# csxmli2016/MARCONet

Measured on AMD Instinct MI355X. Metric: SR images/sec (32x512 LR -> 128x2048 SR), higher is better.
Workload: dtype f16x2; 1 GPU; metric config: batch 256 x 32x512 LR, 16 glyphs/img, enc+TSPGAN+TSPSRNet, fp16x2; per_gpu_batch=256, global_batch=256, glyphs_per_image=16, parallelism=dp1, precision_mode=fp16x2, need_prior_image=True, prior_image_precision=fp16, weights=synthetic:tame, collective=none

## Files before the change

### marconet_amd/_lib.py

```python
import ctypes
import os

_HERE = os.path.dirname(os.path.abspath(__file__))
LIB_PATH = os.environ.get("MARCONET_HIP_LIB", os.path.join(_HERE, "lib", "libmarconet_hip.so"))

ABI_VERSION = 4
MNET_F32, MNET_F16, MNET_F16X2, MNET_F16M = 0, 1, 2, 3
ACT_NONE, ACT_RELU, ACT_LRELU, ACT_LRELU_SQRT2, ACT_TANH, ACT_GELU, ACT_SIGMOID = range(7)
ALGO_AUTO, ALGO_REG_STAGED, ALGO_LDS_DMA, ALGO_SKINNY, ALGO_DMA_CFG0, ALGO_STRIP_CFG0, ALGO_DMA_CFG16, ALGO_FLAG_ONE_TILE = 0, 1, 2, 3, 16, 32, 64, 256
ALGO_FLAG_X1_CENTER = 512
ALGO_FLAG_SHUFFLE2 = 1024

c_int, c_void_p, c_float, c_double, c_i64 = ctypes.c_int32, ctypes.c_void_p, ctypes.c_float, ctypes.c_double, ctypes.c_int64


class ConvDesc(ctypes.Structure):
    _fields_ = [
        ("dtype", c_int),
        ("x0", c_void_p), ("c0", c_int),
        ("x1", c_void_p), ("c1", c_int),
        ("n", c_int), ("h", c_int), ("w", c_int),
        ("wgt", c_void_p),
        ("cout", c_int), ("kh", c_int), ("kw", c_int), ("stride_h", c_int), ("stride_w", c_int),
        ("pad_h", c_int), ("pad_w", c_int),
# ... 34 lines not shown


class CmpStats(ctypes.Structure):
    _fields_ = [("max_abs_diff", c_float), ("max_abs_ref", c_float), ("max_abs_mode", c_float), ("reserved", c_int),
                ("argmax_index", c_i64), ("sum_sq_diff", c_double), ("sum_sq_ref", c_double),
                ("nonfinite_mode", c_i64), ("nonfinite_ref", c_i64)]


CMP_WG_ELEMS, CMP_MAX_SLICES = 2048, 32


def cmp_slices(elems_per_group):
    return max(1, min(CMP_MAX_SLICES, -(-int(elems_per_group) // CMP_WG_ELEMS)))


def cmp_workspace_bytes(n_groups, elems_per_group):
    return int(n_groups) * cmp_slices(elems_per_group) * ctypes.sizeof(CmpStats)


def cmp_records(raw):
    raw = bytes(memoryview(raw).cast("B")) if not isinstance(raw, (bytes, bytearray)) else bytes(raw)
    n = ctypes.sizeof(CmpStats)
    if len(raw) % n:
        raise ValueError("cmp_records: %d bytes are no whole number of %d-byte records" % (len(raw), n))
    return [CmpStats.from_buffer_copy(raw, k) for k in range(0, len(raw), n)]


SYMBOLS = {
    "mnet_last_error": (ctypes.c_char_p, []),
    "mnet_abi_version": (c_int, []),
    "mnet_conv2d_nhwc": (c_int, [ctypes.POINTER(ConvDesc), c_void_p]),
    "mnet_conv2d_nhwc_ex": (c_int, [ctypes.POINTER(ConvDesc), c_int, c_void_p]),
    "mnet_conv2d_splitk": (c_int, [ctypes.POINTER(ConvDesc), c_int, c_void_p, c_void_p]),
    "mnet_conv2d_plan": (c_int, [ctypes.POINTER(ConvDesc), c_int]),
    "mnet_conv2d_flops": (c_double, [ctypes.POINTER(ConvDesc)]),
    "mnet_nchw_to_nhwc": (c_int, [c_void_p, c_void_p, c_int, c_int, c_int, c_int, c_int, c_int, c_void_p]),
    "mnet_nhwc_to_nchw": (c_int, [c_void_p, c_int, c_void_p, c_int, c_int, c_int, c_int, c_int, c_void_p]),
    "mnet_upsample2x_nhwc": (c_int, [c_void_p, c_void_p, c_int, c_int, c_int, c_int, c_int, c_void_p]),
    "mnet_upsample2x_scale_nhwc": (c_int, [c_void_p, c_void_p, c_int, c_int, c_int, c_int, c_int, c_void_p, c_void_p]),
    "mnet_upsample2x_convert_nhwc": (c_int, [c_void_p, c_int, c_void_p, c_int, c_int, c_int, c_int, c_int, c_void_p, c_void_p]),
    "mnet_affine_act_nhwc": (c_int, [c_void_p, c_void_p, c_int, c_int, c_int, c_int, c_void_p, c_void_p, c_int, c_void_p]),
    "mnet_groupnorm_affine": (c_int, [c_void_p, c_int, c_int, c_int, c_int, c_int, c_void_p, c_void_p, c_void_p,
                                      c_float, c_void_p, c_int, c_void_p, c_void_p, c_void_p]),
    "mnet_groupnorm_affine_from_partial": (c_int, [c_void_p, c_int, c_int, c_int, c_int, c_void_p, c_void_p, c_void_p, c_float, c_void_p, c_void_p, c_void_p]),
    "mnet_polyphase_ring_fix": (c_int, [c_void_p, c_void_p, c_void_p, c_void_p, c_void_p, c_int, c_int, c_int, c_int, c_int, c_void_p, c_void_p]),
    "mnet_groupnorm_affine_from_partial_ring": (c_int, [c_void_p, c_void_p, c_int, c_int, c_int, c_int, c_void_p, c_void_p, c_float, c_void_p, c_void_p, c_void_p]),
    "mnet_adain_crop_concat": (c_int, [c_void_p, c_void_p, c_void_p, c_int, c_int, c_int, c_int, c_int,
                                       c_void_p, c_void_p, c_void_p, c_void_p, c_void_p]),
    "mnet_adain_crop_concat_gn": (c_int, [c_void_p, c_void_p, c_void_p, c_int, c_int, c_int, c_int, c_int,
                                          c_void_p, c_void_p, c_void_p, c_void_p, c_void_p, c_void_p, c_float, c_void_p, c_void_p, c_void_p]),
    "mnet_adain_crop_concat_split": (c_int, [c_void_p, c_void_p, c_void_p, c_int, c_int, c_int, c_int, c_int,
                                             c_void_p, c_void_p, c_void_p, c_void_p, c_void_p, c_void_p, c_float, c_void_p, c_void_p,
                                             c_void_p, c_void_p, c_int, c_void_p]),
    "mnet_glyph_scatter_affine": (c_int, [c_void_p, c_void_p, c_void_p, c_void_p, c_int, c_int, c_int, c_int, c_int,
                                          c_void_p, c_void_p, c_void_p, c_void_p]),
    "mnet_layernorm": (c_int, [c_void_p, c_void_p, c_void_p, c_void_p, c_int, c_int, c_float, c_void_p]),
    "mnet_token_mix": (c_int, [c_void_p, c_void_p, c_void_p, c_void_p, c_void_p, c_void_p, c_int, c_int, c_int,
                               c_int, c_float, c_void_p]),
    "mnet_attention": (c_int, [c_void_p, c_void_p, c_int, c_int, c_int, c_float, c_void_p]),
    "mnet_pixelnorm": (c_int, [c_void_p, c_void_p, c_int, c_int, c_void_p]),
    "mnet_embed_gather": (c_int, [c_void_p, c_void_p, c_void_p, c_int, c_int, c_int, c_int, c_int, c_void_p]),
    "mnet_embed_gather_scaled": (c_int, [c_void_p, c_void_p, c_void_p, c_void_p, c_int, c_int, c_int, c_int, c_int, c_void_p]),
    "mnet_demod": (c_int, [c_void_p, c_void_p, c_void_p, c_int, c_int, c_int, c_void_p]),
    "mnet_argmax_rows": (c_int, [c_void_p, c_void_p, c_int, c_int, c_void_p]),
    "mnet_convert": (c_int, [c_void_p, c_int, c_void_p, c_int, c_i64, c_void_p]),
    "mnet_fused_bias_act": (c_int, [c_void_p, c_void_p, c_void_p, c_i64, c_int, c_int, c_float, c_float, c_void_p]),
    "mnet_torgb": (c_int, [c_void_p, c_int, c_int, c_int, c_int, c_int, c_void_p, c_void_p, c_void_p, c_void_p, c_void_p, c_void_p, c_void_p]),
    "mnet_conv3x3_rgb": (c_int, [c_void_p, c_int, c_int, c_int, c_int, c_int, c_void_p, c_void_p, c_int, c_void_p, c_void_p, c_void_p]),
    "mnet_sr_postprocess": (c_int, [c_void_p, c_int, c_void_p, c_int, c_i64, c_int, c_void_p]),
    "mnet_nonfinite_flag": (c_int, [c_void_p, c_int, c_i64, c_void_p, c_void_p]),
    "mnet_compare_stats": (c_int, [c_void_p, c_int, c_void_p, c_int, c_int, c_i64, c_void_p, c_void_p, c_void_p]),
    "mnet_lq_from_u8": (c_int, [c_void_p, c_void_p, c_int, c_int, c_int, c_void_p, c_int, c_void_p]),
    "mnet_panel_u8": (c_int, [c_void_p, c_int, c_void_p, c_int, c_void_p, c_void_p, c_void_p, c_int, c_int, c_void_p, c_void_p]),
    "mnet_stitch_u8": (c_int, [c_void_p, c_int, c_int, c_int, c_void_p, c_void_p, c_int, c_int, c_void_p, c_void_p]),
    "mnet_paste_u8": (c_int, [c_void_p, c_int, c_int, c_int, c_void_p, c_int, c_void_p, c_int, c_int, c_void_p]),
    "mnet_pack_weights": (c_int, [c_void_p, c_int, c_int, c_int, c_int, c_void_p, c_void_p, c_float, c_int, c_int, c_int, c_void_p,
                                  c_void_p, c_void_p]),
    "mnet_pack_wsq": (c_int, [c_void_p, c_int, c_int, c_int, c_float, c_void_p, c_void_p]),
    "mnet_demod_scaled": (c_int, [c_void_p, c_void_p, c_void_p, c_int, c_int, c_int, c_void_p, c_void_p]),
    "mnet_style_rows": (c_int, [c_void_p, c_int, c_int, c_int, c_int, c_void_p, c_int, c_void_p, c_void_p, c_void_p, c_int, c_void_p]),
    "mnet_gather_rows": (c_int, [c_void_p, c_int, c_int, c_int, c_int, c_void_p, c_int, c_void_p, c_void_p]),
}

_lib = None


class MarconetHipError(RuntimeError):
    """Raised for a non-zero C-ABI status; test_sr.py's ``try/except ... continue`` (:181-190) still works."""


def load():
    global _lib
    if _lib is not None:
        return _lib
    if not os.path.isfile(LIB_PATH):
        raise ImportError(
            "marconet_amd: %s not found — build it with `python -c 'import __graft_entry__ as g; g.build()'` "
            "or marconet_amd/csrc/build.sh (there is no CPU/eager fallback)" % LIB_PATH)
    lib = ctypes.CDLL(LIB_PATH)
    for name, (res, args) in SYMBOLS.items():
        fn = getattr(lib, name)
        fn.restype = res
        fn.argtypes = args
    if lib.mnet_abi_version() != ABI_VERSION:
        raise ImportError("marconet_amd: ABI version mismatch in %s" % LIB_PATH)
    _lib = lib
    return lib


def check(status, what):
    if status != 0:
        msg = load().mnet_last_error()
        raise MarconetHipError("%s failed (status %d): %s" % (what, status, msg.decode() if msg else "?"))
```

### marconet_amd/networks.py

```python
import math
import os

import torch
import torch.nn as nn

from . import _lib, ops
from .glyphs import GlyphTables
from .packing import (MX_DTYPE, PRECISIONS, SPLIT_DTYPE, PackCache, is_split, default_precision, equal_linear_scale, pack_conv_weight,
                      pack_linear_weight, pack_polyphase_conv_weight, pack_vec, pack_wsq, padded_cout, rgb_pad, torch_dtype)
from .resnet import resnet45stride as resnet45
from .textvit_arch import TextViT as TextEncoder

_STYLE_NORM = not bool(int(os.environ.get("MNET_NO_STYLE_NORM", "0")))
_FOLD_SKIP = not bool(int(os.environ.get("MNET_NO_FOLD_SKIP", "0")))
_NO_POLYPHASE = os.environ.get("MNET_NO_POLYPHASE", "0") == "1"
_POLYPHASE_CONV_UP = os.environ.get("MNET_POLYPHASE_CONV_UP", "0") == "1"
_FUSE_IMG_CONVERT = os.environ.get("MNET_NO_FUSE_IMG_CONVERT", "0") != "1"
_FUSE_CONV1_MOD = os.environ.get("MNET_NO_FUSE_CONV1_MOD", "0") != "1"
RGB_PAD = 8


class _Precision:
    def set_precision(self, precision):
        if precision not in PRECISIONS:
            raise ValueError("precision must be one of %s" % ", ".join(PRECISIONS))
        self.precision = precision
        for m in self.children():
            if hasattr(m, "precision"):
                m.precision = precision
        return self


class TextContextEncoderV2(nn.Module, _Precision):

    def __init__(self, dim=512, num_classes=6736):
        super().__init__()
        self.resnet = resnet45()
        self.transformer = TextEncoder(num_classes=num_classes, dim=512, max_length=16)
        self.set_precision(default_precision())

    @staticmethod
    def resnet_precision(precision):
        return "fp16x3" if precision == "fp16x2" else precision

    def set_precision(self, precision):
        _Precision.set_precision(self, precision)
        self.resnet.precision = self.resnet_precision(precision)
        return self

    def forward(self, lq, *, precision=None):
        with torch.no_grad(), ops.on_device(lq):
            rp = self.resnet_precision(self.precision if precision is None else precision)
            dtype = torch_dtype(rp)
            x = ops.nchw_to_nhwc(lq.contiguous().float(), dtype, c_ld=rgb_pad(dtype))
            feat = self.resnet.forward_nhwc(x, rp)
            feat = ops.convert(feat, torch.float32)
            return self.transformer.forward_nhwc(feat)


class PixelNorm(nn.Module):
    pass


class EqualLinear(nn.Module):
    def __init__(self, in_channels, out_channels, bias=True, bias_init_val=0, lr_mul=1, activation=None):
        super().__init__()
        self.in_channels, self.out_channels, self.lr_mul, self.activation = in_channels, out_channels, lr_mul, activation
        self.scale = equal_linear_scale(in_channels, lr_mul)
        self.weight = nn.Parameter(torch.randn(out_channels, in_channels).div_(lr_mul))
        if bias:
            self.bias = nn.Parameter(torch.zeros(out_channels).fill_(bias_init_val))
        else:
            self.register_parameter("bias", None)


class SelectText(nn.Module):
    def __init__(self, class_num, channel, size=4):
        super().__init__()
        self.size = size
        self.TextEmbeddings = nn.Parameter(torch.randn(class_num, channel, 1, 1))


class ModulatedConv2d(nn.Module):
    def __init__(self, in_channel, out_channel, kernel_size, style_dim, demodulate=True, upsample=False,
                 downsample=False, blur_kernel=(1, 3, 3, 1)):
        super().__init__()
        self.eps = 1e-8
        self.kernel_size, self.in_channel, self.out_channel = kernel_size, in_channel, out_channel
        self.upsample, self.downsample, self.demodulate = upsample, downsample, demodulate
        self.scale = 1 / math.sqrt(in_channel * kernel_size ** 2)
        self.padding = kernel_size // 2
        self.weight = nn.Parameter(torch.randn(1, out_channel, in_channel, kernel_size, kernel_size))
        self.modulation = EqualLinear(style_dim, in_channel, bias=True, bias_init_val=1, lr_mul=1, activation=None)


class FusedLeakyReLU(nn.Module):

    def __init__(self, channel, negative_slope=0.2, scale=2 ** 0.5):
        super().__init__()
        self.bias = nn.Parameter(torch.zeros(channel))
        self.negative_slope, self.scale = negative_slope, scale


class StyledConv(nn.Module):
    def __init__(self, in_channel, out_channel, kernel_size, style_dim, upsample=False, blur_kernel=(1, 3, 3, 1),
                 demodulate=True):
        super().__init__()
        self.conv = ModulatedConv2d(in_channel, out_channel, kernel_size, style_dim, upsample=upsample,
                                    blur_kernel=blur_kernel, demodulate=demodulate)
        self.bias = nn.Parameter(torch.zeros(1, out_channel, 1, 1))
        self.activate = FusedLeakyReLU(out_channel)


class ToRGB(nn.Module):
    def __init__(self, in_channel, style_dim, upsample=True, blur_kernel=(1, 3, 3, 1)):
        super().__init__()
        self.upsample = upsample
        self.conv = ModulatedConv2d(in_channel, 3, 1, style_dim, demodulate=False)
        self.bias = nn.Parameter(torch.zeros(1, 3, 1, 1))


def returned_image_precision(mode):
    return "fp16x3" if mode == "fp16x2" else None


class TextGenerator(nn.Module):

    def __init__(self, size, style_dim, n_mlp, class_num, channel_multiplier=1, blur_kernel=(1, 3, 3, 1), lr_mlp=0.01):
        super().__init__()
        self.size, self.n_mlp, self.style_dim, self.class_num = size, n_mlp, style_dim, class_num
        self.style_mlp = nn.Sequential(PixelNorm(), *[
            EqualLinear(style_dim, style_dim, bias=True, bias_init_val=0, lr_mul=lr_mlp, activation="fused_lrelu")
            for _ in range(n_mlp)])
        cm = channel_multiplier
        self.channels = {4: 512, 8: 512, 16: 512, 32: 512, 64: 256 * cm, 128: 128 * cm, 256: 64 * cm, 512: 32 * cm,
                         1024: 16 * cm}
        self.input_text = SelectText(class_num, self.channels[4])
        self.conv1 = StyledConv(self.channels[4], self.channels[4], 3, style_dim, blur_kernel=blur_kernel)
        self.to_rgb1 = ToRGB(self.channels[4], style_dim, upsample=False)
        self.log_size = int(math.log(size, 2))
        self.convs, self.upsamples, self.to_rgbs = nn.ModuleList(), nn.ModuleList(), nn.ModuleList()
        cin = self.channels[4]
        for i in range(3, self.log_size + 1):
            cout = self.channels[2 ** i]
            self.convs.append(StyledConv(cin, cout, 3, style_dim, upsample=True, blur_kernel=blur_kernel))
            self.convs.append(StyledConv(cout, cout, 3, style_dim, blur_kernel=blur_kernel))
            self.to_rgbs.append(ToRGB(cout, style_dim))
            cin = cout
        self.n_latent = self.log_size * 2 - 2
        self.precision = default_precision()
        self.module_call_fp16x3 = True
        self._cache = PackCache()

    def _build(self, dtype):
        pk = {}
        f = lambda t: t.detach().float().contiguous()
        pk["mlp"] = []
        for i in range(1, self.n_mlp + 1):
            el = self.style_mlp[i]
            pk["mlp"].append((pack_linear_weight(el.weight, el.scale), f(el.bias.detach() * el.lr_mul)))
        pk["emb"] = f(self.input_text.TextEmbeddings.detach().reshape(self.class_num, -1))

        def styled(sc):
            mc = sc.conv
            w0 = mc.weight.detach()[0]
            return dict(cin=mc.in_channel, cout=mc.out_channel, up=mc.upsample,
                        w=pack_conv_weight(w0, dtype, scale=mc.scale),
                        wsq_t=pack_wsq(w0, mc.scale),
                        mod_w=pack_linear_weight(mc.modulation.weight, mc.modulation.scale), mod_b=f(mc.modulation.bias),
                        bias=f(sc.bias.detach().reshape(-1) + sc.activate.bias.detach()))

        def torgb(tr):
            mc = tr.conv
            return dict(cin=mc.in_channel, w=pack_conv_weight(mc.weight.detach()[0], torch.float32, cin_mult=1, cout_mult=1, scale=mc.scale).reshape(3, -1).contiguous(),
                        mod_w=pack_linear_weight(mc.modulation.weight, mc.modulation.scale), mod_b=f(mc.modulation.bias),
                        bias=pack_vec(tr.bias, 4))

        pk["conv1"] = styled(self.conv1)
        pk["rgb1"] = torgb(self.to_rgb1)
        pk["convs"] = [styled(c) for c in self.convs]
        pk["rgbs"] = [torgb(t) for t in self.to_rgbs]
        layers = [pk["conv1"], pk["rgb1"]] + pk["convs"] + pk["rgbs"]
        off = 0
        for L in layers:
            L["mod_off"] = off
            off += L["cin"]
        pk["mod_all_w"] = torch.cat([L["mod_w"] for L in layers], dim=0).contiguous()
        pk["mod_all_b"] = torch.cat([L["mod_b"] for L in layers], dim=0).contiguous()
        pk["mod_total"] = off
        return pk

    @staticmethod
    def _mod(mod, L, per_glyph=True, bcast=0):
        S, idx = mod[0], mod[1] if per_glyph else None
        if _STYLE_NORM:
            return ops.style_rows(S, L["mod_off"], L["cin"], idx, bcast)
        return ops.gather_rows(S, L["mod_off"], L["cin"], idx), None, None

    @classmethod
    def _style(cls, mod, L):
        s, eps, _ = cls._mod(mod, L)
        if mod[1] is None:
            return s, ops.demod(s, L["wsq_t"], eps)
        su, eps_u, _ = cls._mod(mod, L, per_glyph=False)
        return s, ops.gather_rows(ops.demod(su, L["wsq_t"], eps_u), idx=mod[1])

    @staticmethod
    def _styled(L, x, s, d, premodulated, post=None, out=None):
        return ops.conv2d(x, L["w"], L["cout"], 3, 3, (1, 1), (1, 1), in_scale=None if premodulated else s,
                          out_scale=d, bias=L["bias"], act=ops.ACT_LRELU_SQRT2, post_scale=post, out=out)

    @classmethod
    def _to_rgb(cls, mod, L, x, skip):
        s, _, sb = cls._mod(mod, L, bcast=1)
        return ops.torgb(x, L["w"], s, sb, L["bias"], skip)

    def forward_nhwc(self, styles, labels, need_image=True, style_index=None, p64_out=None, p32_out=None, image_precision=None,
                     precision=None):
        precision = self.precision if precision is None else precision
        pk = self._cache.get(self, precision, self._build)
        dtype = torch_dtype(precision)
        pk_img = pk if image_precision in (None, precision) else self._cache.get(self, image_precision, self._build)
        lat = ops.pixelnorm(styles)
        for w, b in pk["mlp"]:
            lat = ops.linear(lat, w, self.style_dim, bias=b, act=ops.ACT_LRELU_SQRT2)
        mod = (ops.linear(lat, pk["mod_all_w"], pk["mod_total"], bias=pk["mod_all_b"]), style_index)
        s, d = self._style(mod, pk["conv1"])
        x = ops.embed_gather(pk["emb"], labels, dtype, self.class_num, scale=s if _FUSE_CONV1_MOD else None)
        x = self._styled(pk["conv1"], x, s, d, premodulated=_FUSE_CONV1_MOD)
        skip = self._to_rgb(mod, pk["rgb1"], x, None) if need_image else None
        p64 = p32 = None
        for lvl in range(len(pk["rgbs"])):
            if not need_image and p64 is not None and p32 is not None:
                return None, p64, p32
            pkl, up_dtype = pk, None
            if pk_img is not pk and p64 is not None and p32 is not None:
                pkl = pk_img
                up_dtype = torch_dtype(image_precision)
                if not (_FUSE_IMG_CONVERT and up_dtype == torch.float16 and is_split(x.dtype)):
                    x = ops.convert(x, up_dtype)
            La, Lb = pkl["convs"][2 * lvl], pkl["convs"][2 * lvl + 1]
            sa, da = self._style(mod, La)
            sb, db = self._style(mod, Lb)
            xu = ops.upsample2x(x, scale=sa, out_dtype=up_dtype if up_dtype != x.dtype else None)
            xa = self._styled(La, xu, sa, da, premodulated=True, post=sb)
            del xu
            wx = xa.shape[2]
            x = self._styled(Lb, xa, sb, db, premodulated=True, out=p64_out if wx == 64 else (p32_out if wx == 32 else None))
            del xa
            if need_image:
                skip = self._to_rgb(mod, pk["rgbs"][lvl], x, skip)
            if x.shape[2] == 64:
                p64 = x
            if x.shape[2] == 32:
                p32 = x
        if p64 is None or p32 is None:
            raise RuntimeError("no generator level is 64 / 32 pixels wide for %d characters per sample "
                               "(models/networks.py:155-160 selects the prior levels by absolute width)" % labels.shape[1])
        return skip, p64, p32

    def forward(self, styles, labels, noise=None, *, precision=None):
        with torch.no_grad(), ops.on_device(styles):
            styles = styles.contiguous().float()
            labels = labels.to(styles.device).contiguous().long()
            if labels.dim() != 2 or labels.shape[0] != styles.shape[0]:
                raise ValueError("labels must be [N,c] with N == styles.size(0)")
            if labels.numel() and (int(labels.min()) < 0 or int(labels.max()) >= self.class_num):
                raise RuntimeError("label index out of range [0,%d)" % self.class_num)
            mode = self.precision if precision is None else precision
            if mode == "fp16x2" and self.module_call_fp16x3:
                mode = "fp16x3"
            img, p64, p32 = self.forward_nhwc(styles, labels, precision=mode)
            out = ops.nhwc_to_nchw(img, c=3), ops.nhwc_to_nchw(p64), ops.nhwc_to_nchw(p32)
            out[1]._mnet_nhwc, out[2]._mnet_nhwc = (p64, out[1]._version, out[1].data_ptr()), (p32, out[2]._version, out[2].data_ptr())
            return out


class TSPGAN(nn.Module, _Precision):
    def __init__(self, out_size=128, num_style_feat=512, class_num=6736, num_mlp=8):
        super().__init__()
        self.TextGenerator = TextGenerator(size=out_size, style_dim=num_style_feat, n_mlp=num_mlp, class_num=class_num)
        self.precision = default_precision()

    def forward(self, styles, labels, noise):
        return self.TextGenerator(styles, labels, noise, precision=self.precision)


class _SNConv(nn.Module):

    def __init__(self, cin, cout, k=3, stride=1):
        super().__init__()
        self.in_channels, self.out_channels, self.kernel_size, self.stride = cin, cout, k, stride
        conv = nn.Conv2d(cin, cout, k, stride, k // 2)
        self.bias = nn.Parameter(conv.bias.detach().clone())
        self.weight_orig = nn.Parameter(conv.weight.detach().clone())
        nrm = lambda t: t / (t.norm() + 1e-12)
        self.register_buffer("weight_u", nrm(torch.randn(cout)))
        self.register_buffer("weight_v", nrm(torch.randn(cin * k * k)))


def GroupNorm(in_channels):
    assert in_channels % 32 == 0
    return nn.GroupNorm(num_groups=in_channels // 32, num_channels=in_channels, eps=1e-6, affine=True)


def _as_rows32(x):
    b, c = x.shape[:2]
    flat = x.contiguous().float().reshape(b * c, -1)
    m = flat.shape[1]
    mp = (m + 31) // 32 * 32
    if mp != m:
        flat = torch.cat([flat, flat.new_zeros((flat.shape[0], mp - m))], dim=1)
    return flat.reshape(b * c, 1, mp // 32, 32), m, mp


def swish(x):
    v = x.contiguous().float().reshape(1, -1)
    m = v.shape[1]
    mp = (m + 31) // 32 * 32
    if mp != m:
        v = torch.cat([v, v.new_zeros((1, mp - m))], dim=1)
    one = torch.ones((1, 32), dtype=torch.float32, device=x.device)
    y = ops.affine_act(v.reshape(1, 1, mp // 32, 32), one, None, swish=True)
    return y.reshape(-1)[:m].reshape(x.shape)


def calc_mean_std_4D(feat, eps=1e-5):
    if feat.dim() != 4:
        raise AssertionError("The input feature should be 4D tensor.")
# ... 268 lines not shown
```

### marconet_amd/ops.py

```python
import ctypes
import functools
import os

import numpy as np
import torch

from . import _lib
from ._lib import (ACT_GELU, ACT_LRELU, ACT_LRELU_SQRT2, ACT_NONE, ACT_RELU, ACT_SIGMOID, ACT_TANH, MNET_F16,
                   MNET_F16M, MNET_F16X2, MNET_F32, ConvDesc)
from .packing import MX_DTYPE, SPLIT_DTYPE, is_split, mx_weight_rows, new_tensor, tag, untag

__all__ = ["conv2d", "linear", "nchw_to_nhwc", "nhwc_to_nchw", "upsample2x", "affine_act", "groupnorm_affine",
           "adain_crop_concat", "adain_crop_concat_gn", "glyph_scatter_affine", "layernorm", "token_mix", "attention", "pixelnorm",
           "embed_gather", "demod", "argmax_rows", "convert", "fused_bias_act", "sr_postprocess", "lq_from_u8", "panel_u8", "paste_u8", "conv3x3_rgb", "torgb", "stats",
           "pack_weights", "pack_wsq", "gather_rows", "style_rows", "nonfinite_flag", "compare_stats", "gn_partial_buffer", "can_emit_gn_partial", "groupnorm_affine_from_partial",
           "polyphase_plan", "upconv3x3_polyphase", "polyphase_ring_fix", "groupnorm_affine_from_partial_ring",
           "ACT_NONE", "ACT_RELU", "ACT_LRELU", "ACT_LRELU_SQRT2", "ACT_TANH", "ACT_GELU", "ACT_SIGMOID"]


def _plumbing(fn):
    @functools.wraps(fn)
    def wrapper(*args, **kwargs):
        with torch._C.DisableTorchFunctionSubclass():
            return fn(*args, **kwargs)
    return wrapper


def _dt(t):
    if t.dtype == torch.float32:
        return MNET_F32
    if t.dtype == torch.float16:
        return MNET_F16
    if t.dtype == SPLIT_DTYPE:
        return MNET_F16X2
    if t.dtype == MX_DTYPE:
        return MNET_F16M
    raise TypeError("marconet_amd: unsupported dtype %s" % t.dtype)


def _p(t):
    return None if t is None else ctypes.c_void_p(t.data_ptr())


def _addr(t):
    return None if t is None else t.data_ptr()


def _stream():
    return ctypes.c_void_p(torch.cuda.current_stream().cuda_stream)


def _need_cuda(*ts):
    cur = None
    for t in ts:
        if t is None:
            continue
        if not t.is_cuda:
            raise RuntimeError("marconet_amd: tensors must live on a HIP device (got %s); there is no CPU path" % t.device)
        if cur is None:
            cur = torch.cuda.current_device()
        if t.device.index != cur:
            raise RuntimeError("marconet_amd: tensor on %s but the current device is cuda:%d — enter torch.cuda.device(...) "
                               "(the nn.Module forwards and MarconetPipeline do)" % (t.device, cur))
        if not t.is_contiguous():
            raise RuntimeError("marconet_amd: non-contiguous tensor passed to a kernel wrapper")


def _raw(t):
    return untag(t).view(torch.float16) if is_split(t.dtype) else t


@_plumbing
def cat_rows(parts):
    if len(parts) == 1:
        return parts[0]
    out = torch.cat([_raw(p) for p in parts], dim=0)
    return tag(out.view(parts[0].dtype)) if is_split(parts[0].dtype) else out


@_plumbing
def take_rows(t, idx):
    out = _raw(t).index_select(0, idx)
    return tag(out.view(t.dtype)) if is_split(t.dtype) else out


def on_device(t):
    if not t.is_cuda:
        raise RuntimeError("marconet_amd: tensors must live on a HIP device (got %s); there is no CPU path" % t.device)
    return torch.cuda.device(t.device)


class _Stats:

    def __init__(self):
        self.enabled = False
        self.timing = False
        self.reset()

    def reset(self):
# ... 174 lines not shown
    scale = torch.empty((n, c), dtype=torch.float32, device=x.device)
    shift = torch.empty((n, c), dtype=torch.float32, device=x.device)
    stats.tail("groupnorm_stats", (x,), lambda: _lib.check(lib.mnet_groupnorm_affine(_p(x), _dt(x), n, h, w, c, _p(valid_w), _p(gamma), _p(beta), eps,
                                                                                  _p(partial), slices, _p(scale), _p(shift), _stream()), "mnet_groupnorm_affine"))
    return scale, shift


def gn_partial_buffer(n, h, w, c, device):
    return torch.empty((n * h * w // 32, c // 32, 2), dtype=torch.float32, device=device)


_PLAN_CACHE = {}
_PLAN_ADDR = 1 << 20


def _align(t):
    return None if t is None else (128 if t.data_ptr() % 128 == 0 else 16 if t.data_ptr() % 16 == 0 else 0)


def conv_plan(x0, cout, kh=1, kw=1, stride=(1, 1), pad=(0, 0), x1=None, act=ACT_NONE, in_scale=False, residual=False, out_scale=False,
              gn_partial=False, x1_center=False, algo=0):
    n, h, w, c0 = x0.shape
    if x1_center:
        algo |= _lib.ALGO_FLAG_X1_CENTER
    key = (_dt(x0), n, h, w, c0, None if x1 is None else x1.shape[3], _align(x0), _align(x1), cout, kh, kw, tuple(stride), tuple(pad), act,
           bool(in_scale), bool(residual), bool(out_scale), bool(gn_partial), algo)
    k = _PLAN_CACHE.get(key)
    if k is None:
        addr = [_PLAN_ADDR if present else None for present in (in_scale, residual, out_scale, gn_partial)]
        d = _conv_desc(x0, x1, cout, kh, kw, stride, pad, wgt=_PLAN_ADDR, y=_PLAN_ADDR, in_scale=addr[0], residual=addr[1], out_scale=addr[2],
                       act=act, gn_partial=addr[3])
        k = int(_lib.load().mnet_conv2d_plan(ctypes.byref(d), algo))
        if k >= 0:
            _PLAN_CACHE[key] = k
    return k


def polyphase_plan(x, c, act=ACT_NONE, gn_partial=True, algo=0):
    if x.dtype != MX_DTYPE:
        return -1
    return conv_plan(x, 4 * c, 3, 3, (1, 1), (1, 1), act=act, gn_partial=gn_partial, algo=algo | _lib.ALGO_FLAG_SHUFFLE2)


@_plumbing
def polyphase_ring_fix(top, bottom, left, right, y):
    lib = _lib.load()
    _need_cuda(top, bottom, left, right, y)
    n, h2, w2, c = y.shape
    if tuple(top.shape) != (n, 4, w2, c) or tuple(bottom.shape) != (n, 4, w2, c) or tuple(left.shape) != (n, h2, 4, c) or tuple(right.shape) != (n, h2, 4, c):
        raise RuntimeError("polyphase_ring_fix: strips %s %s %s %s do not fit y %s" % (tuple(top.shape), tuple(bottom.shape), tuple(left.shape), tuple(right.shape), tuple(y.shape)))
    sums = torch.empty((n, c // 32, 2), dtype=torch.float64, device=y.device)
    stats.tail("polyphase_ring", (top, left, top, left), lambda: _lib.check(lib.mnet_polyphase_ring_fix(_p(top), _p(bottom), _p(left), _p(right), _p(y), _dt(y), n, h2, w2, c,
                                                                                                      _p(sums), _stream()), "mnet_polyphase_ring_fix"))
    return sums


def groupnorm_affine_from_partial_ring(partial, ring_sums, n, h, w, c, gamma, beta, eps=1e-6):
    lib = _lib.load()
    _need_cuda(partial, ring_sums, gamma, beta)
    scale = torch.empty((n, c), dtype=torch.float32, device=partial.device)
    shift = torch.empty((n, c), dtype=torch.float32, device=partial.device)
    _lib.check(lib.mnet_groupnorm_affine_from_partial_ring(_p(partial), _p(ring_sums), n, h, w, c, _p(gamma), _p(beta), eps, _p(scale), _p(shift), _stream()),
               "mnet_groupnorm_affine_from_partial_ring")
    return scale, shift


@_plumbing
def _strip_pair(x, dim):
    r = _raw(x)
    k = r.shape[dim]
    out = torch.cat([r.narrow(dim, 0, 2), r.narrow(dim, k - 2, 2)], dim=0)
    return tag(out.view(x.dtype)) if is_split(x.dtype) else out


def upconv3x3_polyphase(x, wgt_poly, bias_poly, wgt, bias, c, act=ACT_NONE, algo=0, out=None):
    n, h, w, _ = x.shape
    part = gn_partial_buffer(n, h, w, 4 * c, x.device)
    y = conv2d(x, wgt_poly, 4 * c, 3, 3, (1, 1), (1, 1), bias=bias_poly, act=act, gn_partial=part, algo=algo, shuffle2=True, out=out)
    tb = conv2d(upsample2x(_strip_pair(x, 1)), wgt, c, 3, 3, (1, 1), (1, 1), bias=bias, act=act)
    lr = conv2d(upsample2x(_strip_pair(x, 2)), wgt, c, 3, 3, (1, 1), (1, 1), bias=bias, act=act)
    return y, part, polyphase_ring_fix(tb[:n], tb[n:], lr[:n], lr[n:], y)


def plan_is_lds_dma(k):
    return _lib.ALGO_DMA_CFG0 <= k < _lib.ALGO_STRIP_CFG0 or k >= _lib.ALGO_DMA_CFG16


def can_emit_gn_partial(x0, x1, cout, stride, ho, wo, act=ACT_NONE):
    c = x0.shape[3] + (0 if x1 is None else x1.shape[3])
    if not (x0.dtype == MX_DTYPE and tuple(stride) == (1, 1) and cout >= 64 and cout % 32 == 0 and c % 32 == 0 and x0.shape[3] % 32 == 0
            and (ho * wo) % 32 == 0 and not _NO_EPILOGUE_GN):
        return False
    return conv_plan(x0, cout, 3, 3, stride, (1, 1), x1=x1, act=act, gn_partial=True) >= _lib.ALGO_DMA_CFG0


def groupnorm_affine_from_partial(partial, n, h, w, c, gamma, beta, eps=1e-6, valid_w=None):
    lib = _lib.load()
    _need_cuda(partial, gamma, beta, valid_w)
    scale = torch.empty((n, c), dtype=torch.float32, device=partial.device)
    shift = torch.empty((n, c), dtype=torch.float32, device=partial.device)
    _lib.check(lib.mnet_groupnorm_affine_from_partial(_p(partial), n, h, w, c, _p(valid_w), _p(gamma), _p(beta), eps, _p(scale), _p(shift), _stream()),
               "mnet_groupnorm_affine_from_partial")
    return scale, shift


@_plumbing
def adain_crop_concat(prior, feat, g_img, g_x1, g_y1, g_w):
    lib = _lib.load()
    _need_cuda(prior, feat, g_img, g_x1, g_y1, g_w)
    G, S, S2, C = prior.shape
    B, FH, FW, FC = feat.shape
    if S != S2 or FH != S or FC != C or prior.dtype != feat.dtype:
        raise RuntimeError("adain_crop_concat: shape mismatch prior %s feat %s" % (tuple(prior.shape), tuple(feat.shape)))
    out = new_tensor((G, S, S, 2 * C), prior.dtype, prior.device)
    _lib.check(lib.mnet_adain_crop_concat(_p(prior), _p(feat), _p(out), _dt(prior), G, S, C, FW, _p(g_img), _p(g_x1),
                                          _p(g_y1), _p(g_w), _stream()), "mnet_adain_crop_concat")
    return out


_NO_EPILOGUE_GN = os.environ.get("MNET_NO_EPILOGUE_GN", "0") == "1"
ADAIN_SPLIT_BELOW = 256
_ADAIN_SPLIT = {"0": False, "1": True}.get(os.environ.get("MNET_ADAIN_SPLIT", ""))


@_plumbing
def adain_crop_concat_gn(prior, feat, g_img, g_x1, g_y1, g_w, gamma, beta, eps=1e-6, split=None):
    lib = _lib.load()
    _need_cuda(prior, feat, g_img, g_x1, g_y1, g_w, gamma, beta)
    G, S, S2, C = prior.shape
    B, FH, FW, FC = feat.shape
    if S != S2 or FH != S or FC != C or prior.dtype != feat.dtype or gamma.numel() != 2 * C:
        raise RuntimeError("adain_crop_concat_gn: shape mismatch prior %s feat %s" % (tuple(prior.shape), tuple(feat.shape)))
    out = new_tensor((G, S, S, 2 * C), prior.dtype, prior.device)
    scale = torch.empty((G, 2 * C), dtype=torch.float32, device=prior.device)
    shift = torch.empty((G, 2 * C), dtype=torch.float32, device=prior.device)
    if split is None:
        split = _ADAIN_SPLIT if _ADAIN_SPLIT is not None else G < ADAIN_SPLIT_BELOW
    if split:
        slices = 16
        partial = torch.empty((G * slices * C * 4,), dtype=torch.float64, device=prior.device)
        stat = torch.empty((G, 4, C), dtype=torch.float32, device=prior.device)
        stats.tail("adain", (prior, prior, out), lambda: _lib.check(lib.mnet_adain_crop_concat_split(
            _p(prior), _p(feat), _p(out), _dt(prior), G, S, C, FW, _p(g_img), _p(g_x1), _p(g_y1), _p(g_w), _p(gamma), _p(beta), eps, _p(scale), _p(shift),
            _p(partial), _p(stat), slices, _stream()), "mnet_adain_crop_concat_split"))
        return out, scale, shift
    stats.tail("adain", (prior, prior, out), lambda: _lib.check(lib.mnet_adain_crop_concat_gn(
        _p(prior), _p(feat), _p(out), _dt(prior), G, S, C, FW, _p(g_img), _p(g_x1), _p(g_y1), _p(g_w), _p(gamma), _p(beta), eps, _p(scale), _p(shift), _stream()),
        "mnet_adain_crop_concat_gn"))
    return out, scale, shift


@_plumbing
def glyph_scatter_affine(feat, scale, shift, g_start, g_x1, g_w):
    lib = _lib.load()
    _need_cuda(feat, scale, shift, g_start, g_x1, g_w)
    B, S, FW, C = feat.shape
    out = tag(torch.empty_like(feat))
    stats.tail("glyph_scatter", (feat, scale, shift, out), lambda: _lib.check(lib.mnet_glyph_scatter_affine(
        _p(feat), _p(scale), _p(shift), _p(out), _dt(feat), B, S, C, FW, _p(g_start), _p(g_x1), _p(g_w), _stream()), "mnet_glyph_scatter_affine"))
    return out


def layernorm(x, gamma, beta, eps=1e-5):
    lib = _lib.load()
    _need_cuda(x, gamma, beta)
    rows, d = x.shape
# ... 306 lines not shown
```

### marconet_amd/packing.py

```python
import math
import os
import warnings

import torch

warnings.filterwarnings("ignore", message="ComplexHalf support is experimental")
SPLIT_DTYPE = torch.complex32
MX_DTYPE = torch.uint32
SPLIT_WSCALE = 256.0
PRECISIONS = ("fp32", "fp16", "fp16x3", "fp16x2")
HALF_PRECISIONS = ("fp16", "fp16x3", "fp16x2")


_TAG_GUARD = os.environ.get("MARCONET_TAG_GUARD", "1") != "0"


class BlockedTensor(torch.Tensor):

    _ALLOWED = frozenset((
        "__get__", "__getitem__", "__len__", "__repr__", "__str__", "__format__", "__deepcopy__", "__reduce_ex__", "__hash__",
        "view", "reshape", "contiguous", "flatten", "unsqueeze", "squeeze", "narrow", "select", "index_select", "cat", "stack",
        "chunk", "split", "unbind", "expand", "clone", "detach", "copy_", "to", "cpu", "cuda", "pin_memory", "data_ptr", "numel",
        "dim", "size", "stride", "element_size", "storage_offset", "untyped_storage", "is_contiguous", "get_device", "equal",
        "empty_like", "zeros_like", "new_empty", "new_zeros", "zero_", "record_stream", "is_floating_point", "is_complex",
# ... 63 lines not shown
    return 32 if is_split(dtype) else 8


def split_halves(t):
    if t.shape[-1] % 32 != 0:
        raise ValueError("split-half tensors need a multiple of 32 channels, got %d" % t.shape[-1])
    t = t.detach().float().contiguous()
    hi = t.to(torch.float16)
    if not bool(torch.isfinite(hi).all()):
        raise OverflowError("value %.3g does not fit the half range of the fp16x3 mode" % float(t.abs().max()))
    lo = (t - hi.float()).to(torch.float16)
    blk = t.shape[:-1] + (t.shape[-1] // 32, 32)
    both = torch.stack((hi.reshape(blk), lo.reshape(blk)), dim=-2).contiguous()
    return tag(both.view(SPLIT_DTYPE).reshape(t.shape))


def to_float(t):
    t = untag(t)
    if t.dtype == SPLIT_DTYPE:
        return unsplit_halves(t)
    if t.dtype == MX_DTYPE:
        from . import mxfmt
        return mxfmt.unpack_act(t.contiguous().view(torch.uint8), t.shape[-1])
    return t.float()


def from_float(t, dtype):
    if dtype == SPLIT_DTYPE:
        return split_halves(t)
    if dtype == MX_DTYPE:
        from . import mxfmt
        return tag(mxfmt.pack_act(t).view(MX_DTYPE))
    return t.to(dtype)


def unsplit_halves(t):
    t = untag(t)
    c = t.shape[-1]
    h = t.contiguous().view(torch.float16).reshape(t.shape[:-1] + (c // 32, 2, 32)).float()
    return (h[..., 0, :] + h[..., 1, :]).reshape(t.shape)


def _round_up(v, m):
    return (v + m - 1) // m * m


def padded_cout(o, dtype, cout_mult=4):
    return _round_up(o, max(cout_mult, 32) if is_split(dtype) else cout_mult)


def pack_conv_weight(w, dtype, cin_mult=8, cout_mult=4, scale=1.0, sn=None):
    o, i, kh, kw = w.shape
    if is_split(dtype):
        cin_mult, cout_mult = max(cin_mult, 32), max(cout_mult, 32)
    op, ip = _round_up(o, cout_mult), _round_up(i, cin_mult)
    if w.is_cuda:
        from . import ops
        with ops.on_device(w):
            out = ops.pack_weights(w, dtype, op, ip, scale, None if sn is None else sn[0], None if sn is None else sn[1])
            if is_split(dtype):
                nblk = op * kh * kw * ip // 32
                hi = untag(out).contiguous().view(torch.uint8).reshape(-1)[: nblk * 128].reshape(nblk, 128)[:, :64].contiguous().view(torch.float16)
                if not bool(torch.isfinite(hi).all()):
                    raise OverflowError("a conv weight does not fit the half range of the %s mode (|256 W| >= 65504)"
                                        % ("fp16x3" if dtype == SPLIT_DTYPE else "fp16x2"))
            return out
    w = w.detach().float()
    if sn is not None:
        w = sn_fold(w, sn[0], sn[1])
    if scale != 1.0:
        w = w * scale
    if op != o or ip != i:
        wp = torch.zeros((op, ip, kh, kw), dtype=w.dtype, device=w.device)
        wp[:o, :i] = w
        w = wp
    if dtype == SPLIT_DTYPE:
        return split_halves(w.permute(0, 2, 3, 1).contiguous() * SPLIT_WSCALE)
    if dtype == MX_DTYPE:
        from . import mxfmt
        return mx_weight_tensor(mxfmt.pack_weight(w.permute(0, 2, 3, 1).contiguous()), op, kh, kw, ip)
    return w.permute(0, 2, 3, 1).contiguous().to(dtype)


POLYPHASE_TAPS = (((0.75, 0.25, 0.0), (0.25, 0.75, 0.75), (0.0, 0.0, 0.25)),
                  ((0.25, 0.0, 0.0), (0.75, 0.75, 0.25), (0.0, 0.25, 0.75)))


def polyphase_weight(w):
    o, kh, kw, i = w.shape
    if (kh, kw) != (3, 3):
        raise ValueError("polyphase_weight: 3x3 filters only (got %dx%d)" % (kh, kw))
    w64 = w.detach().to("cpu", torch.float64)
    out = torch.zeros((4, o, 3, 3, i), dtype=torch.float64)
    for py in range(2):
        for px in range(2):
            for a in range(3):
                for r in range(3):
                    ca = POLYPHASE_TAPS[py][a][r]
                    if ca == 0.0:
                        continue
                    for b in range(3):
                        for q in range(3):
                            cb = POLYPHASE_TAPS[px][b][q]
                            if cb != 0.0:
                                out[2 * py + px, :, a, b, :] += (ca * cb) * w64[:, r, q, :]
    return out.reshape(4 * o, 3, 3, i)


def pack_polyphase_conv_weight(w_folded, dtype):
    wp = polyphase_weight(w_folded).to(torch.float32).permute(0, 3, 1, 2).contiguous().to(w_folded.device)
    return pack_conv_weight(wp, dtype)


def mx_weight_rows(cout_pad, kh, kw, cin_pad):
    row_bytes = kh * kw * cin_pad * 4
    return cout_pad + (cout_pad + row_bytes - 1) // row_bytes


def mx_weight_tensor(flat_u8, cout_pad, kh, kw, cin_pad):
    rows = mx_weight_rows(cout_pad, kh, kw, cin_pad)
    buf = torch.zeros((rows * kh * kw * cin_pad * 4,), dtype=torch.uint8, device=flat_u8.device)
    buf[: flat_u8.numel()] = flat_u8
    return tag(buf.view(MX_DTYPE).reshape(rows, kh, kw, cin_pad))


def pack_linear_weight(w, scale=1.0):
    if w.is_cuda:
        from . import ops
        with ops.on_device(w):
            return ops.pack_weights(w, torch.float32, scale=scale).reshape(w.shape[0], w.shape[1])
    return (w.detach().float() * scale).contiguous()


def pack_wsq(w, scale):
    if w.is_cuda:
        from . import ops
        with ops.on_device(w):
            return ops.pack_wsq(w, scale)
    ws = w.detach().float() * scale
    return (ws * ws).sum(dim=(2, 3)).t().contiguous()


def pack_vec(b, n_pad=None):
    b = b.detach().reshape(-1).float()
    if n_pad is not None and n_pad != b.numel():
        bp = torch.zeros((n_pad,), dtype=torch.float32, device=b.device)
        bp[: b.numel()] = b
        b = bp
    return b.contiguous()


def sn_fold(weight_orig, u, v):
    wm = weight_orig.detach().reshape(weight_orig.shape[0], -1)
    sigma = torch.dot(u.detach(), torch.mv(wm, v.detach()))
    return weight_orig.detach() / sigma


class PackCache:

    def __init__(self):
        self._sig = None
        self._store = {}

    @staticmethod
    def signature(module):
        return tuple((t.data_ptr(), t._version, t.device) for t in list(module.parameters()) + list(module.buffers()))

    def get(self, module, precision, builder):
        sig = self.signature(module)
        if sig != self._sig:
            self._store = {}
            self._sig = sig
        if precision not in self._store:
            with torch.no_grad():
                self._store[precision] = builder(torch_dtype(precision))
        return self._store[precision]


def posemb_sincos_1x64(device):
    dim, temperature = 512, 10000
    y, x = torch.meshgrid(torch.arange(1), torch.arange(64), indexing="ij")
    omega = torch.arange(dim // 4) / (dim // 4 - 1)
    omega = 1.0 / (temperature ** omega)
    y = y.flatten()[:, None] * omega[None, :]
    x = x.flatten()[:, None] * omega[None, :]
    pe = torch.cat((x.sin(), x.cos(), y.sin(), y.cos()), dim=1).type(torch.float32)
    return pe.contiguous().to(device)


def equal_linear_scale(in_channels, lr_mul):
    return (1 / math.sqrt(in_channels)) * lr_mul


PACK_FORMAT = "marconet_amd.packed.v2"
PACK_LAYOUT = 6


def _abi_version():
    from . import _lib
    return int(_lib.ABI_VERSION)


def _holders(root):
    return [(name, m) for name, m in root.named_modules() if isinstance(getattr(m, "_cache", None), PackCache) and hasattr(m, "_build")]


def _holder_precision(m):
    return getattr(m, "precision", "fp32")


def _weights_digest(m):
    import hashlib
    h = hashlib.sha256()
    for name, t in list(m.named_parameters()) + list(m.named_buffers()):
        h.update(("%s|%s|%s|" % (name, tuple(t.shape), t.dtype)).encode())
        h.update(t.detach().contiguous().cpu().numpy().tobytes())
    return h.hexdigest()


def _flatten(obj, path, tensors, tree):
    if torch.is_tensor(obj):
        split = is_split(obj.dtype)
        tree[path] = {"t": "tensor", "split": split, "mx": obj.dtype == MX_DTYPE}
        t = untag(obj.detach()).contiguous().cpu()
        tensors[path] = (t.view(torch.float16) if split else t).clone()
    elif isinstance(obj, dict):
        if not all(isinstance(k, str) and "/" not in k for k in obj):
            raise TypeError("packed tree keys must be strings without '/' (at %r)" % path)
        tree[path] = {"t": "dict", "keys": list(obj)}
        for k, v in obj.items():
            _flatten(v, path + "/" + k, tensors, tree)
    elif isinstance(obj, (tuple, list)):
        tree[path] = {"t": "tuple" if isinstance(obj, tuple) else "list", "n": len(obj)}
        for i, v in enumerate(obj):
            _flatten(v, "%s/#%d" % (path, i), tensors, tree)
    elif obj is None or isinstance(obj, (bool, int, float, str)):
        tree[path] = {"t": "py", "v": obj}
    else:
        raise TypeError("cannot serialise %s in a packed tree (at %r)" % (type(obj).__name__, path))


def _unflatten(path, get_tensor, tree):
    node = tree[path]
    if node["t"] == "tensor":
        t = get_tensor(path)
        return tag(t.view(MX_DTYPE if node.get("mx") else SPLIT_DTYPE)) if node.get("split") else t
    if node["t"] == "dict":
        return {k: _unflatten(path + "/" + k, get_tensor, tree) for k in node["keys"]}
    if node["t"] in ("tuple", "list"):
        items = [_unflatten("%s/#%d" % (path, i), get_tensor, tree) for i in range(node["n"])]
        return tuple(items) if node["t"] == "tuple" else items
    return node["v"]


def save_packed(path, **roots):
    import json
    from safetensors.torch import save_file
    tensors, trees, digests = {}, {}, {}
    for rname, root in roots.items():
        for hname, m in _holders(root):
            prec = _holder_precision(m)
            m._cache.get(m, prec, m._build)
            digest = _weights_digest(m)
            for pr in [prec] + sorted(k for k in m._cache._store if k != prec):
                key = "%s|%s" % (rname + ("." + hname if hname else ""), pr)
                flat, tree = {}, {}
                _flatten(m._cache._store[pr], "", flat, tree)
                trees[key] = tree
                digests[key] = digest
                for p, t in flat.items():
                    tensors[key + "|" + p] = t
    if not tensors:
        raise ValueError("save_packed: no packed-weight holders in the given modules")
    save_file(tensors, path, metadata={"format": PACK_FORMAT, "layout": str(PACK_LAYOUT), "abi": str(_abi_version()),
                                       "trees": json.dumps(trees), "weights_sha256": json.dumps(digests)})
    return sorted(trees)


# ... 30 lines not shown
```

Measured before the change: 262.3 images/s.

## Fold bilinear 2x upsample into 3x3 conv via low-res per-tap conv

For the 512-channel upsampling StyleGAN levels, the code no longer upsamples and then runs a 3x3 conv at high resolution. It runs a 1x1 conv at low resolution that emits 9*cout per-tap partial outputs, then a new HIP kernel bilinearly upsamples each tap and sums them, with demod scale, bias, activation and next-layer modulation fused in. This cuts the conv work to roughly a quarter, at the cost of writing and reading a 9x-wide intermediate tensor. The path is limited to the MX storage dtype and to large enough heights, and falls back to the old path otherwise.

After: 272.0 images/s (median of 6 runs). 1.04x the previous value.

```diff
diff --git a/include/marconet_hip_upfold.h b/include/marconet_hip_upfold.h
--- /dev/null
+++ b/include/marconet_hip_upfold.h
@@ -0,0 +1,16 @@
+#ifndef MARCONET_HIP_UPFOLD_H
+#define MARCONET_HIP_UPFOLD_H
+
+#include "marconet_hip.h"
+
+#ifdef __cplusplus
+extern "C" {
+#endif
+
+int mnet_upfold3x3_nhwc(const void* z, void* y, int32_t dtype, int32_t n, int32_t h, int32_t w, int32_t c,
+                        const float* out_scale, const float* bias, int32_t act, const float* post_scale, void* stream);
+
+#ifdef __cplusplus
+}
+#endif
+#endif
diff --git a/marconet_amd/_lib.py b/marconet_amd/_lib.py
--- a/marconet_amd/_lib.py
+++ b/marconet_amd/_lib.py
@@ -140,6 +140,10 @@
     "mnet_gather_rows": (c_int, [c_void_p, c_int, c_int, c_int, c_int, c_void_p, c_int, c_void_p, c_void_p]),
 }
 
+UPFOLD_SYMBOLS = {
+    "mnet_upfold3x3_nhwc": (c_int, [c_void_p, c_void_p, c_int, c_int, c_int, c_int, c_int, c_void_p, c_void_p, c_int, c_void_p, c_void_p]),
+}
+
 _lib = None
 
 
@@ -156,7 +160,7 @@
             "marconet_amd: %s not found — build it with `python -c 'import __graft_entry__ as g; g.build()'` "
             "or marconet_amd/csrc/build.sh (there is no CPU/eager fallback)" % LIB_PATH)
     lib = ctypes.CDLL(LIB_PATH)
-    for name, (res, args) in SYMBOLS.items():
+    for name, (res, args) in list(SYMBOLS.items()) + list(UPFOLD_SYMBOLS.items()):
         fn = getattr(lib, name)
         fn.restype = res
         fn.argtypes = args
diff --git a/marconet_amd/csrc/upfold_kernels.hip b/marconet_amd/csrc/upfold_kernels.hip
--- /dev/null
+++ b/marconet_amd/csrc/upfold_kernels.hip
@@ -0,0 +1,147 @@
+#include "common.h"
+#include "../../include/marconet_hip_upfold.h"
+
+#ifndef MNET_UPF_RUN
+#define MNET_UPF_RUN 8
+#endif
+
+template <typename T>
+__global__ void __launch_bounds__(256, 2) upfold_kernel(const T* __restrict__ z, T* __restrict__ y, int H, int W, int C,
+                                                        const float* __restrict__ out_scale, const float* __restrict__ bias,
+                                                        const float* __restrict__ post_scale, int act, unsigned items_per_image) {
+    constexpr int N = Vec<T>::N;
+    constexpr int R = MNET_UPF_RUN;
+    const unsigned cpp = (unsigned)C / N;
+    unsigned bx = blockIdx.x, by = blockIdx.y;
+    {
+        const unsigned NWG = gridDim.x * gridDim.y, L = by * gridDim.x + bx;
+        if ((NWG & 7u) == 0u) { const unsigned V = (L & 7u) * (NWG >> 3) + (L >> 3); by = V / gridDim.x; bx = V - by * gridDim.x; }
+    }
+    const int n = (int)by;
+    const size_t zpix = (size_t)9 * C;
+    const T* zbase = z + (size_t)n * H * W * zpix;
+    T* ybase = y + (size_t)n * 4 * H * W * C;
+    const int W2 = 2 * W;
+    for (unsigned id = bx * 256u + threadIdx.x; id < items_per_image; id += gridDim.x * 256u) {
+        const unsigned ch = id % cpp, col = id / cpp;
+        const int X = (int)(col % (unsigned)W2), y0 = (int)(col / (unsigned)W2) * R, y1 = min(y0 + R, H);
+        unsigned c0[3], c1[3];
+        float w0[3], w1[3];
+#pragma unroll
+        for (int kx = 0; kx < 3; ++kx) {
+            const int xu = X + kx - 1, xc = min(max(xu, 0), W2 - 1), m = xc >> 1;
+            const bool odd = xc & 1, in = xu >= 0 && xu < W2;
+            c0[kx] = (unsigned)(odd ? m : max(m - 1, 0)) * (unsigned)zpix;
+            c1[kx] = (unsigned)(odd ? min(m + 1, W - 1) : m) * (unsigned)zpix;
+            w0[kx] = in ? (odd ? 0.75f : 0.25f) : 0.f;
+            w1[kx] = in ? (odd ? 0.25f : 0.75f) : 0.f;
+        }
+        const T* base = zbase + (size_t)ch * N;
+        auto hrow = [&](int r, float (&h)[3][N]) __attribute__((always_inline)) {
+            const T* rp = base + (size_t)r * W * zpix;
+#pragma unroll
+            for (int ky = 0; ky < 3; ++ky) {
+#pragma unroll
+                for (int kx = 0; kx < 3; ++kx) {
+                    const T* tp = rp + (size_t)(3 * ky + kx) * C;
+                    float a[N], b[N];
+                    unpackr<T>(ldraw<T>(tp + c0[kx]), a);
+                    unpackr<T>(ldraw<T>(tp + c1[kx]), b);
+#pragma unroll
+                    for (int j = 0; j < N; ++j) {
+                        const float t = w0[kx] * a[j] + w1[kx] * b[j];
+                        h[ky][j] = kx == 0 ? t : h[ky][j] + t;
+                    }
+                }
+                __builtin_amdgcn_sched_barrier(0);
+            }
+        };
+        const float* osp = out_scale ? out_scale + (size_t)n * C + (size_t)ch * N : nullptr;
+        const float* bsp = bias ? bias + (size_t)ch * N : nullptr;
+        const float* psp = post_scale ? post_scale + (size_t)n * C + (size_t)ch * N : nullptr;
+        auto emit1 = [&](T* q, float (&v)[N]) __attribute__((always_inline)) {
+            float o[N];
+#pragma unroll
+            for (int j = 0; j < N; ++j) o[j] = v[j];
+            if (osp) {
+#pragma unroll
+                for (int j = 0; j < N; j += 4) { const f32x4 s4 = *reinterpret_cast<const f32x4*>(osp + j); o[j] *= s4[0]; o[j + 1] *= s4[1]; o[j + 2] *= s4[2]; o[j + 3] *= s4[3]; }
+            }
+            if (bsp) {
+#pragma unroll
+                for (int j = 0; j < N; j += 4) { const f32x4 b4 = *reinterpret_cast<const f32x4*>(bsp + j); o[j] += b4[0]; o[j + 1] += b4[1]; o[j + 2] += b4[2]; o[j + 3] += b4[3]; }
+            }
+            act_apply_vec<N, true>(o, act);
+            if (psp) {
+#pragma unroll
+                for (int j = 0; j < N; j += 4) { const f32x4 p4 = *reinterpret_cast<const f32x4*>(psp + j); o[j] *= p4[0]; o[j + 1] *= p4[1]; o[j + 2] *= p4[2]; o[j + 3] *= p4[3]; }
+            }
+            straw<T>(q, packr<T>(o));
+        };
+        float h[3][N];
+        float e[N], o[N];
+        float ne[N], no[N];
+        hrow(max(y0 - 1, 0), h);
+        {
+            const bool in = y0 > 0;
+#pragma unroll
+            for (int j = 0; j < N; ++j) {
+                e[j] = (in ? 0.75f * h[0][j] : 0.f) + 0.25f * h[1][j];
+                o[j] = 0.25f * h[0][j];
+            }
+        }
+        auto centre = [&](int r) __attribute__((always_inline)) {
+            const bool up = r > 0, dn = r + 1 < H;
+#pragma unroll
+            for (int j = 0; j < N; ++j) {
+                e[j] += ((up ? 0.25f * h[0][j] : 0.f) + 0.75f * h[1][j]) + 0.75f * h[2][j];
+                o[j] += (0.75f * h[0][j] + 0.75f * h[1][j]) + (dn ? 0.25f * h[2][j] : 0.f);
+                ne[j] = 0.75f * h[0][j] + 0.25f * h[1][j];
+                no[j] = 0.25f * h[0][j];
+            }
+        };
+        hrow(y0, h);
+        centre(y0);
+        const size_t orow = (size_t)W2 * C;
+#pragma unroll 1
+        for (int i = y0; i < y1; ++i) {
+            hrow(min(i + 1, H - 1), h);
+            const bool in = i + 1 < H;
+#pragma unroll
+            for (int j = 0; j < N; ++j) {
+                e[j] += 0.25f * h[2][j];
+                o[j] += 0.25f * h[1][j] + (in ? 0.75f * h[2][j] : 0.f);
+            }
+            T* q = ybase + ((size_t)(2 * i) * W2 + X) * C + (size_t)ch * N;
+            emit1(q, e);
+            emit1(q + orow, o);
+            if (i + 1 < y1) {
+#pragma unroll
+                for (int j = 0; j < N; ++j) { e[j] = ne[j]; o[j] = no[j]; }
+                centre(i + 1);
+            }
+        }
+    }
+}
+
+extern "C" int mnet_upfold3x3_nhwc(const void* z, void* y, int32_t dtype, int32_t n, int32_t h, int32_t w, int32_t c,
+                                   const float* out_scale, const float* bias, int32_t act, const float* post_scale, void* stream) {
+    MNET_CHECK_ARG(z && y && z != y, "upfold3x3: null pointer (or y == z: not an in-place kernel)");
+    MNET_CHECK_ARG(n > 0 && n <= 65535 && h > 0 && w > 0 && c > 0, "upfold3x3: bad geometry");
+    MNET_CHECK_ARG(is_storage(dtype), "upfold3x3: bad dtype");
+    MNET_CHECK_ARG(act == MNET_ACT_NONE || act == MNET_ACT_LRELU || act == MNET_ACT_LRELU_SQRT2, "upfold3x3: activation must be NONE, LRELU or LRELU_SQRT2");
+    const int N = chunk_n(dtype);
+    MNET_CHECK_ALIGN(c % N == 0 && aligned16(z) && aligned16(y) && aligned16(out_scale) && aligned16(bias) && aligned16(post_scale),
+                     "upfold3x3: c %% %d != 0 or unaligned", N);
+    MNET_CHECK_ALIGN(!is_split4(dtype) || (c % 32 == 0 && aligned128(z) && aligned128(y)), "upfold3x3: blocked storages need c %% 32 == 0, 128-byte aligned");
+    MNET_CHECK_ARG((long long)h * w * (c / N) * 4 < (1ll << 31) && (long long)w * 9 * c < (1ll << 29), "upfold3x3: image too large");
+    const long long per = (long long)((h + MNET_UPF_RUN - 1) / MNET_UPF_RUN) * 2 * w * (c / N);
+    const int gx = (int)((per + 255) / 256 < 2048 ? (per + 255) / 256 : 2048);
+    hipStream_t st = reinterpret_cast<hipStream_t>(stream);
+    dispatch_storage(dtype, [&](auto tag) {
+        using T = typename decltype(tag)::type;
+        hipLaunchKernelGGL((upfold_kernel<T>), dim3(gx, n), dim3(256), 0, st, (const T*)z, (T*)y, h, w, c, out_scale, bias, post_scale, act, (unsigned)per);
+    });
+    MNET_LAUNCH_CHECK("upfold3x3");
+    return MNET_OK;
+}
diff --git a/marconet_amd/networks.py b/marconet_amd/networks.py
--- a/marconet_amd/networks.py
+++ b/marconet_amd/networks.py
@@ -7,13 +7,14 @@
 from . import _lib, ops
 from .glyphs import GlyphTables
 from .packing import (MX_DTYPE, PRECISIONS, SPLIT_DTYPE, PackCache, is_split, default_precision, equal_linear_scale, pack_conv_weight,
-                      pack_linear_weight, pack_polyphase_conv_weight, pack_vec, pack_wsq, padded_cout, rgb_pad, torch_dtype)
+                      pack_linear_weight, pack_polyphase_conv_weight, pack_tapconv_weight, pack_vec, pack_wsq, padded_cout, rgb_pad, torch_dtype)
 from .resnet import resnet45stride as resnet45
 from .textvit_arch import TextViT as TextEncoder
 
 _STYLE_NORM = not bool(int(os.environ.get("MNET_NO_STYLE_NORM", "0")))
 _FOLD_SKIP = not bool(int(os.environ.get("MNET_NO_FOLD_SKIP", "0")))
 _NO_POLYPHASE = os.environ.get("MNET_NO_POLYPHASE", "0") == "1"
+_NO_UPFOLD = os.environ.get("MNET_NO_UPFOLD", "0") == "1"
 _POLYPHASE_CONV_UP = os.environ.get("MNET_POLYPHASE_CONV_UP", "0") == "1"
 _FUSE_IMG_CONVERT = os.environ.get("MNET_NO_FUSE_IMG_CONVERT", "0") != "1"
 _FUSE_CONV1_MOD = os.environ.get("MNET_NO_FUSE_CONV1_MOD", "0") != "1"
@@ -166,6 +167,7 @@
             w0 = mc.weight.detach()[0]
             return dict(cin=mc.in_channel, cout=mc.out_channel, up=mc.upsample,
                         w=pack_conv_weight(w0, dtype, scale=mc.scale),
+                        w_tap=pack_tapconv_weight(w0, dtype, scale=mc.scale) if mc.upsample and dtype == MX_DTYPE and (mc.in_channel, mc.out_channel) in ops.UPFOLD_LEVELS else None,
                         wsq_t=pack_wsq(w0, mc.scale),
                         mod_w=pack_linear_weight(mc.modulation.weight, mc.modulation.scale), mod_b=f(mc.modulation.bias),
                         bias=f(sc.bias.detach().reshape(-1) + sc.activate.bias.detach()))
@@ -242,9 +244,16 @@
             La, Lb = pkl["convs"][2 * lvl], pkl["convs"][2 * lvl + 1]
             sa, da = self._style(mod, La)
             sb, db = self._style(mod, Lb)
-            xu = ops.upsample2x(x, scale=sa, out_dtype=up_dtype if up_dtype != x.dtype else None)
-            xa = self._styled(La, xu, sa, da, premodulated=True, post=sb)
-            del xu
+            if La["w_tap"] is not None and up_dtype is None and not _NO_UPFOLD and ops.upfold_plan(x, La["cout"]) >= 0:
+                xs = ops.affine_act(x, sa)
+                z = ops.conv2d(xs, La["w_tap"], 9 * La["cout"], 1, 1)
+                del xs
+                xa = ops.upfold3x3(z, La["cout"], out_scale=da, bias=La["bias"], act=ops.ACT_LRELU_SQRT2, post_scale=sb)
+                del z
+            else:
+                xu = ops.upsample2x(x, scale=sa, out_dtype=up_dtype if up_dtype != x.dtype else None)
+                xa = self._styled(La, xu, sa, da, premodulated=True, post=sb)
+                del xu
             wx = xa.shape[2]
             x = self._styled(Lb, xa, sb, db, premodulated=True, out=p64_out if wx == 64 else (p32_out if wx == 32 else None))
             del xa
diff --git a/marconet_amd/ops.py b/marconet_amd/ops.py
--- a/marconet_amd/ops.py
+++ b/marconet_amd/ops.py
@@ -14,7 +14,7 @@
            "adain_crop_concat", "adain_crop_concat_gn", "glyph_scatter_affine", "layernorm", "token_mix", "attention", "pixelnorm",
            "embed_gather", "demod", "argmax_rows", "convert", "fused_bias_act", "sr_postprocess", "lq_from_u8", "panel_u8", "paste_u8", "conv3x3_rgb", "torgb", "stats",
            "pack_weights", "pack_wsq", "gather_rows", "style_rows", "nonfinite_flag", "compare_stats", "gn_partial_buffer", "can_emit_gn_partial", "groupnorm_affine_from_partial",
-           "polyphase_plan", "upconv3x3_polyphase", "polyphase_ring_fix", "groupnorm_affine_from_partial_ring",
+           "polyphase_plan", "upconv3x3_polyphase", "polyphase_ring_fix", "groupnorm_affine_from_partial_ring", "upfold_plan", "upfold3x3",
            "ACT_NONE", "ACT_RELU", "ACT_LRELU", "ACT_LRELU_SQRT2", "ACT_TANH", "ACT_GELU", "ACT_SIGMOID"]
 
 
@@ -355,6 +355,40 @@
     return y, part, polyphase_ring_fix(tb[:n], tb[n:], lr[:n], lr[n:], y)
 
 
+UPFOLD_LEVELS = {(512, 512): 16, (512, 256): 16}
+
+
+def upfold_plan(x, cout, levels=None):
+    if x.dtype != MX_DTYPE:
+        return -1
+    _, h, _, cin = x.shape
+    min_h = (UPFOLD_LEVELS if levels is None else levels).get((cin, cout))
+    if min_h is None or h < min_h:
+        return -1
+    k = conv_plan(x, 9 * cout, 1, 1)
+    return k if k >= 0 and plan_is_lds_dma(k) else -1
+
+
+@_plumbing
+def upfold3x3(z, c, out_scale=None, bias=None, act=ACT_NONE, post_scale=None, out=None):
+    lib = _lib.load()
+    _need_cuda(z, out_scale, bias, post_scale, out)
+    n, h, w, c9 = z.shape
+    if c9 != 9 * c:
+        raise RuntimeError("upfold3x3: z has %d channels, expected 9 x %d" % (c9, c))
+    for t, nm in ((out_scale, "out_scale"), (bias, "bias"), (post_scale, "post_scale")):
+        if t is not None and t.dtype != torch.float32:
+            raise TypeError("upfold3x3: %s must be float32" % nm)
+    oshape = (n, 2 * h, 2 * w, c)
+    if out is None:
+        out = new_tensor(oshape, z.dtype, z.device)
+    elif tuple(out.shape) != oshape or out.dtype != z.dtype:
+        raise RuntimeError("upfold3x3: out is %s %s, expected %s %s" % (tuple(out.shape), out.dtype, oshape, z.dtype))
+    stats.tail("upfold", (z, out), lambda: _lib.check(lib.mnet_upfold3x3_nhwc(_p(z), _p(out), _dt(z), n, h, w, c, _p(out_scale), _p(bias), act, _p(post_scale),
+                                                                             _stream()), "mnet_upfold3x3_nhwc"))
+    return out
+
+
 def plan_is_lds_dma(k):
     return _lib.ALGO_DMA_CFG0 <= k < _lib.ALGO_STRIP_CFG0 or k >= _lib.ALGO_DMA_CFG16
 
diff --git a/marconet_amd/packing.py b/marconet_amd/packing.py
--- a/marconet_amd/packing.py
+++ b/marconet_amd/packing.py
@@ -169,6 +169,19 @@
     return w.permute(0, 2, 3, 1).contiguous().to(dtype)
 
 
+def tapconv_weight(w):
+    o, i, kh, kw = w.shape
+    if (kh, kw) != (3, 3):
+        raise ValueError("tapconv_weight: 3x3 filters only (got %dx%d)" % (kh, kw))
+    return w.detach().permute(2, 3, 0, 1).reshape(9 * o, i, 1, 1).contiguous()
+
+
+def pack_tapconv_weight(w0, dtype, scale=1.0):
+    if is_split(dtype) and w0.shape[0] % 32 != 0:
+        raise ValueError("pack_tapconv_weight: %d output channels are no whole number of 32-channel blocks" % w0.shape[0])
+    return pack_conv_weight(tapconv_weight(w0), dtype, scale=scale)
+
+
 POLYPHASE_TAPS = (((0.75, 0.25, 0.0), (0.25, 0.75, 0.75), (0.0, 0.0, 0.25)),
                   ((0.25, 0.0, 0.0), (0.75, 0.75, 0.25), (0.0, 0.25, 0.75)))
 
@@ -280,7 +293,7 @@
 
 
 PACK_FORMAT = "marconet_amd.packed.v2"
-PACK_LAYOUT = 6
+PACK_LAYOUT = 7
 
 
 def _abi_version():
```
